# alshai/Big-BWT

Hardware: AMD Instinct MI355X
Metric: input MB/s to .bwt (bit-exact vs ref) (higher is better)
Workload: dtype u8; 1 GPU; BASELINE configs[2]: 64x mutated yeast-shaped FASTA (~0.79 GB), -w 10 -p 100, BWT + -s -e sampled SA; bytes_per_gpu=787308470, w=10, p=100, flags=6, phrases=16409159, words=921010, dict_bytes=79900101, parallelism=1 GPU

## Files before the change

big-bwt_amd/csrc/merge.hip:

```cpp
#include "kernels.hpp"
#include "prims.hpp"
#include "devutil.hpp"
#include <algorithm>
#include <cstdlib>

namespace pfp {

static constexpr int TB = 256;
constexpr int kOffTileLog = 11;


template <class I> struct alignas(16) Idx8 { I v[8]; };
__device__ __forceinline__ void tile_full_count(const uint32_t p8[8], int nk, uint64_t t0, uint32_t *__restrict__ tile_full,
                                                unsigned long long *__restrict__ first_full) {
  __shared__ uint32_t ws[4];
  uint32_t cfull = 0;
  int firstk = -1;
#pragma unroll
  for (int k = 7; k >= 0; k--) if (k < nk && p8[k] == kEndOfWord) { cfull++; firstk = k; }
  const unsigned long long anyf = __ballot(cfull != 0);
  for (int o = 32; o > 0; o >>= 1) cfull += __shfl_down(cfull, o, 64);
  if ((threadIdx.x & 63) == 0) ws[threadIdx.x >> 6] = cfull;
  if (anyf && (int)(threadIdx.x & 63) == __ffsll((long long)anyf) - 1) atomicMin(first_full, (unsigned long long)(t0 + firstk));
  __syncthreads();
// ... 169 lines not shown
__global__ void full_base0_kernel(const unsigned long long *__restrict__ first_full, const I *__restrict__ sa,
                                  WordView wv, const uint32_t *__restrict__ lexrank, uint32_t *__restrict__ out) {
  const unsigned long long f = *first_full;
  *out = f == ~0ull ? 0u : lexrank[word_of(wv, sa[f])];
}

template <class I>
__global__ void group_flags_kernel(uint64_t N, const I *__restrict__ grp, const uint8_t *__restrict__ pc,
                                   int any_multi_is_hard, uint8_t *__restrict__ hard) {
  uint64_t t = (uint64_t)BID * blockDim.x + threadIdx.x;
  if (t >= N || pc[t] == 0) return;
  I g = grp[t];
  if (g == t) return;
  if (any_multi_is_hard || pc[t] != pc[g]) hard[g] = 1;
}

enum : uint8_t { CLS_NONE = 0, CLS_FILL = 1, CLS_FULL = 2, CLS_HARD = 3, CLS_MULTI = 4 };
enum : int { SA_NONE = 0, SA_DENSE = 1, SA_SPARSE = 2 };

template <class I>
__global__ void gather_idx_kernel(uint64_t n, const I *__restrict__ idx, const I *__restrict__ src, I *__restrict__ dst) {
  uint64_t i = (uint64_t)BID * blockDim.x + threadIdx.x;
  if (i < n) dst[i] = src[idx[i]];
}
struct alignas(32) WordRec { uint32_t ist, occ, first, last; uint64_t wend, pad; };
__global__ void wistart_kernel(uint32_t d, const uint32_t *__restrict__ lexrank, const uint32_t *__restrict__ istart_lex,
                               const uint32_t *__restrict__ wocc, const uint32_t *__restrict__ ilist,
                               const uint64_t *__restrict__ wend, uint32_t *__restrict__ wistart, WordRec *__restrict__ wrec) {
  uint32_t j = BID * blockDim.x + threadIdx.x;
  if (j >= d) return;
  const uint32_t st = istart_lex[lexrank[j]] + 1;
  wistart[j] = st;
  if (wrec) { const uint32_t oc = wocc[j]; wrec[j] = WordRec{st, oc, ilist[st], ilist[st + oc - 1], wend[j], 0}; }
}

template <class I>
struct MergeArgsT {
  uint64_t N, n_out; uint32_t d; int w; int want_sa;
  uint64_t pos_base, n_out_global;
  uint64_t out_lo, out_hi;
  const I *sa, *grp;
  WordView wv;
  const uint32_t *ist, *wistart;
  const WordRec *wrec;
  const uint32_t *sfirst, *slast, *ssl;
  const uint8_t *pc, *hard, *gmaj;
  const uint64_t *tbase; const uint32_t *loc;
  const uint32_t *ilist; const uint8_t *bwlast; const uint64_t *bwsai;
  const uint32_t *istart_lex, *fullbase, *fullbase0;
  uint8_t *bwt; uint64_t *out_sa;
  int pass;
  const uint64_t *bmap, *bpre;
  uint64_t *sa_c;
};
enum : int { PASS_BWT = 1, PASS_SA = 2 };
template <class I>
__device__ __forceinline__ void sa_put(const MergeArgsT<I> &a, uint64_t x, uint64_t v) {
  if (x < a.out_lo || x >= a.out_hi) return;
  if (!a.bmap) { a.out_sa[x] = v; return; }
  const uint64_t r = x - a.out_lo, wv = a.bmap[r >> 6];
  if (!((wv >> (r & 63)) & 1ull)) return;
  if (a.sa_c) a.sa_c[a.bpre[r >> 6] + (uint64_t)__popcll(wv & ((1ull << (r & 63)) - 1ull))] = v;
  else a.out_sa[x] = v;
}
template <class I>
__device__ __forceinline__ bool sa_wanted(const MergeArgsT<I> &a, uint64_t x) {
  if (x < a.out_lo || x >= a.out_hi) return false;
  if (!a.bmap) return true;
  const uint64_t r = x - a.out_lo;
  return (a.bmap[r >> 6] >> (r & 63)) & 1ull;
}
template <class I>
__device__ __forceinline__ uint64_t slot_off(const MergeArgsT<I> &a, uint64_t t) { return a.tbase[t >> kOffTileLog] + a.loc[t]; }


__device__ __forceinline__ uint8_t fix_char(uint8_t ch) { return ch == kDollar ? 0 : ch; }
template <class I>
__device__ __forceinline__ uint32_t slot_ist(const MergeArgsT<I> &a, uint64_t t) {
  return a.ist ? a.ist[t] : a.wistart[word_of(a.wv, a.sa[t])];
}

template <class I>
__device__ __forceinline__ uint32_t slot_first(const MergeArgsT<I> &a, uint64_t t) { return a.sfirst ? a.sfirst[t] : a.wrec[word_of(a.wv, a.sa[t])].first; }
template <class I>
__device__ __forceinline__ uint32_t slot_last(const MergeArgsT<I> &a, uint64_t t) { return a.slast ? a.slast[t] : a.wrec[word_of(a.wv, a.sa[t])].last; }
template <class I>
__device__ __forceinline__ uint64_t slot_slen(const MergeArgsT<I> &a, uint64_t t) {
  if (a.ssl) { const uint32_t v = a.ssl[t]; if (v != kSlCap) return v; }
  return slen_of(a.wv, a.sa[t]);
}

constexpr int kHardLds = 1024;
constexpr int kHardRank = 512;
constexpr int kHardMem = 256;
constexpr int kHardSortMin = 512;
constexpr int kSlots = 2048;
constexpr uint64_t kExpandQuota = 1u << 16;

struct ExpandLds {
  uint32_t loff[kSlots + 1];
  uint32_t lfist[kSlots];
  uint8_t lpc[kSlots], lcls[kSlots];
  uint32_t ccnt[kSlots / 64 + 1];
};

template <class I>
// ... 383 lines not shown
          uint32_t lb, pv = 0, sv = 0;
          bool hp = false, hs = false;
          if (m == me) {
            lb = j;
            if (a.want_sa) {
              if (j > 0) { pv = a.ilist[my_ist + j - 1]; hp = true; }
              if (j + 1 < my_occ) { sv = a.ilist[my_ist + j + 1]; hs = true; }
            }
          } else {
            const uint32_t mfirst = slot_first(a, g + m), mlast = slot_last(a, g + m);
            if (pos < mfirst) { lb = 0; sv = mfirst; hs = true; }
            else if (pos > mlast) { lb = (uint32_t)(slot_off(a, g + m + 1) - slot_off(a, g + m)); pv = mlast; hp = true; }
            else {
              const WordRec wr = a.wrec[word_of(a.wv, a.sa[g + m])];
              const uint32_t *lst = a.ilist + wr.ist;
              uint32_t l2 = 1, h2 = wr.occ - 1;
              while (l2 < h2) { const uint32_t mid = (l2 + h2) >> 1; if (lst[mid] < pos) l2 = mid + 1; else h2 = mid; }
              lb = l2;
              if (a.want_sa) { pv = lst[lb - 1]; hp = true; sv = lst[lb]; hs = true; }
            }
          }
          r += lb;
          if (hp && (!has_pred || pv > pred)) { pred = pv; has_pred = 1; }
          if (hs && (!has_succ || sv < succ)) { succ = sv; has_succ = 1; }
        }
      }
#pragma unroll
      for (int o = 1; o < LPM; o <<= 1) {
        r += __shfl_xor(r, o, 64);
        const uint32_t op = __shfl_xor(pred, o, 64), ohp = __shfl_xor(has_pred, o, 64);
        const uint32_t os = __shfl_xor(succ, o, 64), ohs = __shfl_xor(has_succ, o, 64);
        if (ohp && (!has_pred || op > pred)) { pred = op; has_pred = 1; }
        if (ohs && (!has_succ || os < succ)) { succ = os; has_succ = 1; }
      }
      if (!act || ll != 0) continue;
      const uint64_t o = base + r;
      if (o >= a.out_lo && o < a.out_hi) a.bwt[o] = mych;
      if (a.want_sa)
        recs[mmv.roff + j] = MinorRec{o, pos, pred, succ, has_pred | (has_succ << 1), (uint32_t)sl, 0u};
    }
  }
}

template <class I>
__global__ void hard_minor_sa_kernel(MergeArgsT<I> a, const MinorRec *__restrict__ recs, uint64_t n) {
  const uint64_t q = (uint64_t)BID * blockDim.x + threadIdx.x;
  if (q >= n) return;
  const MinorRec r = recs[q];
  sa_put(a, r.o, a.bwsai[r.pos] - (uint64_t)r.sl);
  if ((r.flags & 1u) && r.o >= 1) sa_put(a, r.o - 1, a.bwsai[r.pred] - (uint64_t)r.sl);
  if (r.flags & 2u) sa_put(a, r.o + 1, a.bwsai[r.succ] - (uint64_t)r.sl);
}

struct BigGroup { uint64_t g; uint64_t E; uint32_t k; uint32_t pad; };
struct HardLds {
  uint32_t lpos[kHardRank];
  uint8_t lq[kHardRank];
  uint32_t lmoff[kHardMem + 1], lmist[kHardMem], lmsl[kHardMem];
  uint8_t lmch[kHardMem], lmg[kHardMem];
  uint64_t gbase[64], ghead[64];
  uint32_t geoff[65], gk0[65];
};
__device__ __forceinline__ void wave_lds_sync() {
  __builtin_amdgcn_wave_barrier();
  __threadfence_block();
}
__device__ __forceinline__ uint32_t wave_max_u32(uint32_t v) {
#pragma unroll
  for (int o = 32; o > 0; o >>= 1) { const uint32_t x = __shfl_xor(v, o, 64); v = x > v ? x : v; }
  return v;
}
template <class I>
__global__ __launch_bounds__(256) void hard_groups_kernel(MergeArgsT<I> a, const I *__restrict__ heads,
                                                          const uint64_t *__restrict__ nheads_p,
                                                          unsigned long long *__restrict__ stats,
                                                          BigGroup *__restrict__ big, uint32_t big_cap,
                                                          BigGroup *__restrict__ mid, uint32_t mid_cap, int gpb) {
  __shared__ HardLds S[4];
  const int wv = threadIdx.x >> 6, lane = threadIdx.x & 63;
  HardLds &L = S[wv];
  const uint64_t nH = *nheads_p;
  const uint64_t nbatch = (nH + gpb - 1) / gpb;
  unsigned long long my_chars = 0, my_groups = 0;
  for (uint64_t b = BID * 4 + wv; b < nbatch; b += GDIM * 4) {
    const uint64_t hidx = b * gpb + lane;
    uint64_t g = 0, base = 0;
    uint32_t k = 0, E = 0;
    bool live = false;
    if (lane < gpb && hidx < nH) {
      g = heads[hidx];
      uint32_t kk = 0;
      while (g + kk < a.N && a.grp[g + kk] == (I)g && a.pc[g + kk] != 0) kk++;
      base = slot_off(a, g);
      const uint64_t Eg = slot_off(a, g + kk) - base;
      if (kk && !(base + Eg <= a.out_lo || base >= a.out_hi)) {
        my_chars += Eg; my_groups += 1;
        const bool sorted_path = Eg > (uint64_t)kHardSortMin;
        if (Eg <= (uint64_t)kHardRank && kk <= (uint32_t)kHardMem && !sorted_path) { live = true; k = kk; E = (uint32_t)Eg; }
        else if (Eg <= (uint64_t)kHardLds && sorted_path) {
          const unsigned long long idx = atomicAdd(&stats[3], 1ull);
          if (idx < mid_cap) mid[idx] = BigGroup{g, Eg, kk, 0};
        } else {
          const unsigned long long idx = atomicAdd(&stats[2], 1ull);
          if (idx < big_cap) big[idx] = BigGroup{g, Eg, kk, 0};
        }
      }
    }
    unsigned long long todo = __ballot(live);
    while (todo) {
      const bool mine = (todo >> lane) & 1ull;
      uint32_t pk = mine ? k : 0u, pE = mine ? E : 0u;
#pragma unroll
      for (int o = 1; o < 64; o <<= 1) {
        const uint32_t vk = __shfl_up(pk, o, 64), vE = __shfl_up(pE, o, 64);
        if (lane >= o) { pk += vk; pE += vE; }
      }
      const bool fit = mine && pk <= (uint32_t)kHardMem && pE <= (uint32_t)kHardRank;
      const unsigned long long take = __ballot(fit);
      todo &= ~take;
      const int nG = __popcll(take);
      const int lastl = 63 - __clzll((long long)take);
      const uint32_t M = __shfl(pk, lastl, 64), Eb = __shfl(pE, lastl, 64);
      if (fit) {
        const int gi = __popcll(take & ((1ull << lane) - 1ull));
        L.ghead[gi] = g; L.gbase[gi] = base; L.geoff[gi] = pE - E; L.gk0[gi] = pk - k;
      }
      if (lane == 0) { L.geoff[nG] = Eb; L.gk0[nG] = M; }
      wave_lds_sync();
      for (uint32_t q = lane; q < M; q += 64) {
        int lo = 0, hi = nG;
        while (hi - lo > 1) { const int mid = (lo + hi) >> 1; if (L.gk0[mid] <= q) lo = mid; else hi = mid; }
        const uint64_t t = L.ghead[lo] + (q - L.gk0[lo]);
        L.lmoff[q] = L.geoff[lo] + (uint32_t)(slot_off(a, t) - L.gbase[lo]);
        L.lmist[q] = slot_ist(a, t);
        uint32_t sl = 0;
        if (a.want_sa) sl = (uint32_t)slot_slen(a, t);
        L.lmsl[q] = sl;
        L.lmch[q] = fix_char(a.pc[t]);
        L.lmg[q] = (uint8_t)lo;
      }
      if (lane == 0) L.lmoff[M] = Eb;
      wave_lds_sync();
      for (uint32_t e = lane; e < Eb; e += 64) {
        uint32_t lo = 0, hi = M;
        while (hi - lo > 1) { const uint32_t mid = (lo + hi) >> 1; if (L.lmoff[mid] <= e) lo = mid; else hi = mid; }
        L.lpos[e] = a.ilist[L.lmist[lo] + (e - L.lmoff[lo])];
        L.lq[e] = (uint8_t)lo;
      }
      wave_lds_sync();
      for (uint32_t e = lane; e < Eb; e += 64) {
        const uint32_t q = L.lq[e], gi = L.lmg[q];
        const uint32_t s0 = L.geoff[gi], s1 = L.geoff[gi + 1], k0 = L.gk0[gi], k1 = L.gk0[gi + 1];
        const uint32_t Eg = s1 - s0, kg = k1 - k0;
        const uint32_t pos = L.lpos[e];
        uint32_t lg = 1;
        while ((kg << lg) < Eg) lg++;
        const bool by_search = (uint64_t)kg * (lg + 1) * 3 < Eg;
        uint32_t r = 0;
        if (!by_search) {
          for (uint32_t x = s0; x < s1; x++) r += L.lpos[x] < pos;
        } else {
          for (uint32_t m2 = k0; m2 < k1; m2++) {
            uint32_t l2 = L.lmoff[m2], h2 = L.lmoff[m2 + 1];
            const uint32_t b2 = l2;
            while (l2 < h2) { const uint32_t mid = (l2 + h2) >> 1; if (L.lpos[mid] < pos) l2 = mid + 1; else h2 = mid; }
            r += l2 - b2;
          }
        }
        const uint64_t o = L.gbase[gi] + r;
        if (o >= a.out_lo && o < a.out_hi) {
          if (a.pass & PASS_BWT) a.bwt[o] = L.lmch[q];
          if (a.want_sa && (a.pass & PASS_SA)) sa_put(a, o, a.bwsai[pos] - (uint64_t)L.lmsl[q]);
        }
      }
      wave_lds_sync();
    }
  }
#pragma unroll
  for (int o = 32; o > 0; o >>= 1) { my_chars += __shfl_down(my_chars, o, 64); my_groups += __shfl_down(my_groups, o, 64); }
  if (lane == 0 && (my_chars | my_groups)) { atomicAdd(&stats[0], my_chars); atomicAdd(&stats[1], my_groups); }
}

template <class I>
__global__ __launch_bounds__(256) void hard_sort_kernel(MergeArgsT<I> a, const BigGroup *__restrict__ mid, uint32_t nmid) {
  __shared__ uint64_t skey[4][kHardLds];
  const int wv = threadIdx.x >> 6, lane = threadIdx.x & 63;
  uint64_t *K = skey[wv];
  for (uint32_t qi = BID * 4 + wv; qi < nmid; qi += GDIM * 4) {
    const uint64_t g = mid[qi].g;
    const uint32_t E = (uint32_t)mid[qi].E, k = mid[qi].k;
    const uint64_t base = slot_off(a, g);
    uint32_t n = 64;
    while (n < E) n <<= 1;
    for (uint32_t e = lane; e < n; e += 64) {
      uint64_t key = ~0ull;
      if (e < E) {
        uint32_t lo = 0, hi = k;
        while (hi - lo > 1) { const uint32_t mdl = (lo + hi) >> 1; if (slot_off(a, g + mdl) - base <= e) lo = mdl; else hi = mdl; }
        const uint32_t pos = a.ilist[slot_ist(a, g + lo) + (e - (uint32_t)(slot_off(a, g + lo) - base))];
        key = ((uint64_t)pos << 16) | e;
      }
      K[e] = key;
    }
    wave_lds_sync();
    for (uint32_t k2 = 2; k2 <= n; k2 <<= 1)
      for (uint32_t j = k2 >> 1; j > 0; j >>= 1) {
        for (uint32_t i = lane; i < (n >> 1); i += 64) {
          const uint32_t x = ((i & ~(j - 1)) << 1) | (i & (j - 1)), y = x | j;
          const uint64_t kx = K[x], ky = K[y];
          if ((kx > ky) == ((x & k2) == 0)) { K[x] = ky; K[y] = kx; }
        }
        wave_lds_sync();
      }
    for (uint32_t r = lane; r < E; r += 64) {
      const uint64_t key = K[r];
      const uint32_t pos = (uint32_t)(key >> 16), e = (uint32_t)(key & 0xffffu);
      const uint64_t o = base + r;
      if (o < a.out_lo || o >= a.out_hi) continue;
      uint32_t lo = 0, hi = k;
      while (hi - lo > 1) { const uint32_t mdl = (lo + hi) >> 1; if (slot_off(a, g + mdl) - base <= e) lo = mdl; else hi = mdl; }
      const uint64_t t = g + lo;
      if (a.pass & PASS_BWT) a.bwt[o] = fix_char(a.pc[t]);
      if (a.want_sa && (a.pass & PASS_SA)) sa_put(a, o, a.bwsai[pos] - slot_slen(a, t));
    }
    wave_lds_sync();
  }
}

template <class I>
__global__ __launch_bounds__(256) void hard_big_kernel(MergeArgsT<I> a, const BigGroup *__restrict__ big, uint32_t nbig,
                                                       const uint64_t *__restrict__ estart, uint64_t total) {
  const uint64_t e0 = estart[0];
  for (uint64_t gi = (uint64_t)BID * 256 + threadIdx.x; gi < total; gi += (uint64_t)GDIM * 256) {
    const uint64_t ge = e0 + gi;
    uint32_t lo = 0, hi = nbig;
    while (hi - lo > 1) { uint32_t mid = (lo + hi) >> 1; if (estart[mid] <= ge) lo = mid; else hi = mid; }
    const uint64_t g = big[lo].g, e = ge - estart[lo];
    const uint32_t k = big[lo].k;
    const uint64_t base = slot_off(a, g);
    uint32_t ml = 0, mh = k;
    while (mh - ml > 1) { uint32_t mid = (ml + mh) >> 1; if (slot_off(a, g + mid) - base <= e) ml = mid; else mh = mid; }
    const uint64_t t = g + ml;
    const uint32_t j = (uint32_t)(e - (slot_off(a, t) - base));
    const uint32_t pos = a.ilist[slot_ist(a, t) + j];
    uint64_t r = j;
    for (uint64_t t2 = g; t2 < g + k; t2++) {
      if (t2 == t) continue;
      const uint32_t *lst = a.ilist + slot_ist(a, t2);
      uint32_t l2 = 0, h2 = (uint32_t)(slot_off(a, t2 + 1) - slot_off(a, t2));
      while (l2 < h2) { uint32_t mid = (l2 + h2) >> 1; if (lst[mid] < pos) l2 = mid + 1; else h2 = mid; }
      r += l2;
    }
    if (base + r >= a.out_lo && base + r < a.out_hi) {
      if (a.pass & PASS_BWT) a.bwt[base + r] = fix_char(a.pc[t]);
      if (a.want_sa && (a.pass & PASS_SA)) sa_put(a, base + r, a.bwsai[pos] - slot_slen(a, t));
    }
  }
}

template <class I>
__global__ __launch_bounds__(256) void big_keys_kernel(MergeArgsT<I> a, const BigGroup *__restrict__ big, uint32_t q0, uint32_t q1,
                                                       const uint64_t *__restrict__ estart, uint64_t cnt,
                                                       uint64_t *__restrict__ keys, uint64_t *__restrict__ vals) {
  const uint64_t i = (uint64_t)BID * 256 + threadIdx.x;
  if (i >= cnt) return;
  const uint64_t ge = estart[q0] + i;
  uint32_t lo = q0, hi = q1;
  while (hi - lo > 1) { const uint32_t mid = (lo + hi) >> 1; if (estart[mid] <= ge) lo = mid; else hi = mid; }
  const uint64_t g = big[lo].g, e = ge - estart[lo];
  const uint32_t k = big[lo].k;
  const uint64_t base = slot_off(a, g);
  uint32_t ml = 0, mh = k;
  while (mh - ml > 1) { const uint32_t mid = (ml + mh) >> 1; if (slot_off(a, g + mid) - base <= e) ml = mid; else mh = mid; }
  const uint64_t t = g + ml;
  const uint32_t j = (uint32_t)(e - (slot_off(a, t) - base));
  keys[i] = ((uint64_t)(lo - q0) << 32) | a.ilist[slot_ist(a, t) + j];
  vals[i] = t;
}
template <class I>
__global__ __launch_bounds__(256) void big_place_kernel(MergeArgsT<I> a, const BigGroup *__restrict__ big, uint32_t q0,
                                                        const uint64_t *__restrict__ estart, uint64_t cnt,
                                                        const uint64_t *__restrict__ keys, const uint64_t *__restrict__ vals) {
  const uint64_t i = (uint64_t)BID * 256 + threadIdx.x;
  if (i >= cnt) return;
  const uint64_t key = keys[i], t = vals[i];
  const uint32_t lo = q0 + (uint32_t)(key >> 32), pos = (uint32_t)key;
  const uint64_t o = slot_off(a, big[lo].g) + (estart[q0] + i - estart[lo]);
  if (o < a.out_lo || o >= a.out_hi) return;
  if (a.pass & PASS_BWT) a.bwt[o] = fix_char(a.pc[t]);
  if (a.want_sa && (a.pass & PASS_SA) && sa_wanted(a, o)) sa_put(a, o, a.bwsai[pos] - slot_slen(a, t));
}

__global__ __launch_bounds__(256) void slot_loc_kernel(const uint32_t *__restrict__ cnt, uint64_t N, uint32_t *__restrict__ loc,
                                                       uint64_t *__restrict__ tsum, uint32_t *__restrict__ overflow) {
  __shared__ uint64_t ws[4];
  if (((uint64_t)BID << kOffTileLog) > N) return;
  const uint64_t t0 = ((uint64_t)BID << kOffTileLog) + (uint64_t)threadIdx.x * 8;
  uint32_t v[8];
  if (t0 + 8 <= N) {
    const uint4 x = *reinterpret_cast<const uint4 *>(cnt + t0), y = *reinterpret_cast<const uint4 *>(cnt + t0 + 4);
    v[0] = x.x; v[1] = x.y; v[2] = x.z; v[3] = x.w; v[4] = y.x; v[5] = y.y; v[6] = y.z; v[7] = y.w;
  } else {
    for (int k = 0; k < 8; k++) v[k] = t0 + k < N ? cnt[t0 + k] : 0u;
  }
  uint64_t own = 0;
  for (int k = 0; k < 8; k++) own += v[k];
  uint64_t inc = own;
  const int lane = threadIdx.x & 63, wv = threadIdx.x >> 6;
  for (int o = 1; o < 64; o <<= 1) { const uint64_t u = __shfl_up(inc, o, 64); if (lane >= o) inc += u; }
  if (lane == 63) ws[wv] = inc;
  __syncthreads();
  uint64_t run = inc - own;
  for (int q = 0; q < wv; q++) run += ws[q];
  uint32_t o8[8];
  for (int k = 0; k < 8; k++) { o8[k] = (uint32_t)run; run += v[k]; }
  *reinterpret_cast<uint4 *>(loc + t0) = make_uint4(o8[0], o8[1], o8[2], o8[3]);
  *reinterpret_cast<uint4 *>(loc + t0 + 4) = make_uint4(o8[4], o8[5], o8[6], o8[7]);
  if (threadIdx.x == 255) {
    tsum[BID] = run;
    if (run >> 32) atomicOr(overflow, 1u);
  }
}


enum class RecordSource {
  SortKeys,
  Gathered,
  PerSlot,
};

struct MergeSwitches {
  int prec_direct = -1;
  uint32_t big_cap = 0;
  uint64_t big_budget = 1ull << 27;
  static MergeSwitches read() {
    MergeSwitches s;
    if (const char *e = getenv("PFP_PREC_DIRECT")) s.prec_direct = atoi(e) != 0;
    if (const char *e = getenv("PFP_BIG_CAP")) { if (atoll(e) > 0) s.big_cap = (uint32_t)atoll(e); }
    if (const char *e = getenv("PFP_BIG_BUDGET")) s.big_budget = strtoull(e, nullptr, 10);
    return s;
  }
};

// ... 20 lines not shown
  const Dictionary &D;
  const DictIndex &ix;
  const SuffixOrderT<I> &so;
  const ParseBWT &pb;
  const uint32_t *const occ_lex;
  const MergeOpts o;
  BwtOutputs &out;
  const uint64_t NP, N;
  const uint32_t d;
  const int sa_mode;
  const MergeSwitches sw;
  const RecordSource src;
  const WordView wv;
  const uint64_t ntile;
  const uint32_t nblk;
  const int first_pass;

  MergeArgsT<I> a{};
  uint64_t n_out = 0;

  struct {
    DBuf<uint32_t> istart_lex, wistart;
    DBuf<WordRec> wrec;
  } word;
  struct {
    DBuf<uint8_t> pc, hard;
    DBuf<uint32_t> loc, ovf;
    DBuf<uint64_t> tsum, tbase;
    DBuf<uint32_t> tile_full, fullbase, fullbase0;
    DBuf<unsigned long long> first_full;
    DBuf<uint32_t> sfirst, slast, ssl;
  } slot;
  enum { kAllHeads = 0, kFallbackHeads = 1 };
  struct {
    DBuf<unsigned long long> hstats;
    uint64_t n_heads = 0;
    uint32_t big_cap = 0, mid_cap = 0;
    DBuf<BigGroup> big, mid;
    DBuf<I> heads;
    DBuf<uint64_t> list_len;
    DBuf<unsigned long long> mstat;
    DBuf<uint8_t> gmaj, fallback;
    DBuf<HardGroupInfo> ginfo;
    DBuf<uint32_t> minor_cnt, mm_cnt;
    DBuf<uint64_t> minor_off, mm_off;
    DBuf<MinorMember> mm_list;
    uint64_t n_mm = 0, sum_k = 0, n_minor = 0;
    DBuf<I> fb_heads;
    DBuf<MinorRec> recs;
    int gpb = 64;
    uint32_t nmid = 0, nbig = 0;
    DBuf<uint64_t> estart;
    std::vector<uint64_t> es;
  } hg;
  DBuf<uint32_t> heavy, nheavy;

  Merge(pfp_ctx *c_, const Dictionary &D_, const DictIndex &ix_, const SuffixOrderT<I> &so_, const ParseBWT &pb_, const uint32_t *occ_lex_,
        const MergeOpts &o_, BwtOutputs &out_)
      : c(c_), D(D_), ix(ix_), so(so_), pb(pb_), occ_lex(occ_lex_), o(o_), out(out_), NP(D_.dsize), N(so_.N), d((uint32_t)D_.d),
        sa_mode(!o_.flags ? SA_NONE : ((o_.flags & PFP_FLAG_SA) ? SA_DENSE : SA_SPARSE)), sw(MergeSwitches::read()),
        src(choose_record_source<I>(c_, N, NP, sa_mode, so_, sw)), wv(word_view(D_, ix_)), ntile((N >> kOffTileLog) + 1),
        nblk((uint32_t)cdiv64(N, kSlots)), first_pass(sa_mode == SA_SPARSE ? PASS_BWT : (PASS_BWT | PASS_SA)) {}

  MergeArgsT<I> with_pass(int pass) const { MergeArgsT<I> x = a; x.pass = pass; return x; }

  void word_records() {
    word.istart_lex.alloc(c, d); word.wistart.alloc(c, d);
    exclusive_sum_u32(c, occ_lex, word.istart_lex.p, d);
    word.wrec.alloc(c, d);
    hipLaunchKernelGGL(wistart_kernel, gdim(cdiv(d, TB)), gdim(TB), 0, c->stream, d, ix.lexrank.p, word.istart_lex.p, D.wocc.p, pb.ilist.p,
                       ix.wend.p, word.wistart.p, word.wrec.p);
  }

  void alloc_slot_tables() {
    slot.pc.alloc(c, N + 8); slot.hard.alloc(c, N);
    slot.loc.alloc(c, ntile << kOffTileLog); slot.ovf.alloc(c, 1);
    alloc_counts(c, slot.tsum, ntile); slot.tbase.alloc(c, ntile + 1);
    slot.hard.zero();
    slot.tile_full.alloc(c, ntile + 1); slot.fullbase.alloc(c, ntile + 1); slot.fullbase0.alloc(c, 1);
    slot.first_full.alloc(c, 1);
    slot.tile_full.zero();
    PFP_HIP(hipMemsetAsync(slot.first_full.p, 0xFF, 8, c->stream));
    slot.ovf.zero();
  }
  void slot_tables_from_keys(DBuf<uint32_t> &cnt) {
    { KScope ks(c, "pfp::slot_payload_kernel", N * (8 + 1 + 5));
      hipLaunchKernelGGL(slot_payload_kernel<I>, gdim(cdiv(cdiv64(N, 8), 256)), gdim(256), 0, c->stream, N, so.sa.p, so.skeys.p,
                         so.refined.p, D.bytes.p, wv, D.wocc.p, d, o.w, cnt.p, slot.pc.p, slot.tile_full.p, slot.first_full.p); }
    { KScope ks(c, "pfp::slot_loc_kernel", N * 8);
      hipLaunchKernelGGL(slot_loc_kernel, gdim((unsigned)ntile), gdim(256), 0, c->stream, cnt.p, N, slot.loc.p, slot.tsum.p, slot.ovf.p); }
    { KScope ks(c, "pfp::group_flags_kernel", N * 5);
      hipLaunchKernelGGL(group_flags_kernel<I>, gdim(cdiv(N, TB)), gdim(TB), 0, c->stream, N, so.grp.p, slot.pc.p, 0, slot.hard.p); }
  }
  void slot_tables_gathered() {
    const int dense = sa_mode == SA_DENSE ? 1 : 0;
    const uint64_t np256 = cdiv64(NP, 256) * 256;
    DBuf<PosRec> prec(c, np256);
    { KScope ks(c, "pfp::pprec16_kernel", NP * (1 + 16) + (uint64_t)d * 40);
      hipLaunchKernelGGL(pprec16_kernel, gdim(cdiv(np256, TB)), gdim(TB), 0, c->stream, wv, o.w, reinterpret_cast<const uint4 *>(word.wrec.p),
                         dense, (uint64_t)0, NP, prec.p); }
    slot_records(prec.p);
  }
  void slot_tables_per_slot() { slot_records(nullptr); }
  void slot_records(const PosRec *prec) {
    const int dense = sa_mode == SA_DENSE ? 1 : 0;
    slot.sfirst.alloc(c, ntile << kOffTileLog);
// ... 25 lines not shown
    a.ist = dense ? slot.sfirst.p : nullptr;
    a.wistart = word.wistart.p; a.wrec = word.wrec.p;
    a.sfirst = dense ? nullptr : slot.sfirst.p; a.slast = slot.slast.p; a.ssl = slot.ssl.p;
    a.pc = slot.pc.p; a.hard = slot.hard.p; a.tbase = slot.tbase.p; a.loc = slot.loc.p;
    a.ilist = pb.ilist.p; a.bwlast = pb.bwlast.p; a.bwsai = pb.bwsai.p;
    a.istart_lex = word.istart_lex.p; a.fullbase = slot.fullbase.p; a.fullbase0 = slot.fullbase0.p;
    a.out_lo = o.out_lo; a.out_hi = o.out_hi < n_out ? o.out_hi : n_out;
    a.bwt = out.d_bwt - o.out_lo; a.out_sa = out.d_sa ? out.d_sa - o.out_lo : nullptr;
  }

  void find_hard_groups() {
    hg.hstats.alloc(c, 5);
    hg.hstats.zero();
    hg.n_heads = count_flags(c, slot.hard.p, N);
    hg.big_cap = sw.big_cap ? sw.big_cap : (uint32_t)std::min<uint64_t>({(uint64_t)1u << 20, hg.n_heads + 1, n_out / 1024 + 1});
    hg.big.alloc(c, hg.big_cap);
    hg.mid_cap = (uint32_t)std::min<uint64_t>(n_out / (kHardSortMin + 1) + 64, 0x7FFFFFFFull);
    hg.mid.alloc(c, hg.mid_cap);
    hg.heads.alloc(c, hg.n_heads + 1);
    hg.list_len.alloc(c, 2);
    select_index<I>(c, slot.hard.p, hg.heads.p, hg.list_len.p + kAllHeads, N);
    hg.mstat.alloc(c, 2);
    hg.mstat.zero();
  }

  HeadList<I> classify() {
    const uint64_t n_heads = hg.n_heads;
    hg.gmaj.alloc(c, N); hg.fallback.alloc(c, n_heads); hg.ginfo.alloc(c, n_heads);
    alloc_counts(c, hg.minor_cnt, n_heads); hg.minor_off.alloc(c, n_heads + 1);
    alloc_counts(c, hg.mm_cnt, n_heads); hg.mm_off.alloc(c, n_heads + 1);
    a.gmaj = hg.gmaj.p;
    { KScope ks(c, "pfp::hard_classify_kernel", n_heads * 40);
      hipLaunchKernelGGL(hard_classify_kernel<I>, gdim(cdiv(n_heads, 256)), gdim(256), 0, c->stream, a, hg.heads.p, n_heads, hg.gmaj.p,
                         hg.ginfo.p, hg.minor_cnt.p, hg.fallback.p, hg.mstat.p, hg.mm_cnt.p); }
    exclusive_sum_u32_u64(c, hg.minor_cnt.p, hg.minor_off.p, n_heads + 1);
    exclusive_sum_u32_u64(c, hg.mm_cnt.p, hg.mm_off.p, n_heads + 1);
    hg.n_mm = read_scalar(c, hg.mm_off.p + n_heads);
    hg.sum_k = read_scalar(c, (const uint64_t *)hg.mstat.p + 1);
    if (hg.n_mm) {
      hg.mm_list.alloc(c, hg.n_mm);
      KScope ks(c, "pfp::hard_minor_fill_kernel", n_heads * 40 + hg.n_mm * 16);
      hipLaunchKernelGGL(hard_minor_fill_kernel<I>, gdim(cdiv(n_heads * 8, 256)), gdim(256), 0, c->stream, a, hg.ginfo.p, n_heads, hg.mm_off.p,
                         hg.minor_off.p, hg.gmaj.p, hg.mm_list.p);
    }
    const uint64_t n_fallback = count_flags(c, hg.fallback.p, n_heads);
    hg.n_minor = read_scalar(c, hg.minor_off.p + n_heads);
    hg.fb_heads.alloc(c, n_fallback + 1);
    {
      DBuf<I> fidx(c, n_fallback + 1);
      select_index<I>(c, hg.fallback.p, fidx.p, hg.list_len.p + kFallbackHeads, n_heads);
      if (n_fallback) hipLaunchKernelGGL(gather_idx_kernel<I>, gdim(cdiv(n_fallback, 256)), gdim(256), 0, c->stream, n_fallback, fidx.p,
                                         hg.heads.p, hg.fb_heads.p);
      PFP_HIP(hipGetLastError());
      sync(c);
    }
    return HeadList<I>{hg.fb_heads.p, hg.list_len.p + kFallbackHeads, n_fallback};
  }

  void expand() {
    const MergeArgsT<I> ap = with_pass(first_pass);
    heavy.alloc(c, nblk); nheavy.alloc(c, 1);
    nheavy.zero();
    { KScope ks(c, "pfp::expand_kernel", N * 14 + n_out * (sa_mode == SA_DENSE ? 17 : 1));
      hipLaunchKernelGGL(expand_kernel<I>, gdim(nblk), gdim(256), 0, c->stream, ap, heavy.p, nheavy.p, nblk); }
    const uint32_t nh = read_scalar(c, nheavy.p);
    KScope ks2(c, "pfp::expand_heavy_kernel", 0);
    if (nh) hipLaunchKernelGGL(expand_heavy_kernel<I>, gdim(c->n_cu * 4), gdim(256), 0, c->stream, ap, heavy.p, nh);
    PFP_HIP(hipGetLastError());
  }

  void place_minority(const HeadList<I> &lds) {
    if (hg.n_mm) {
      const MergeArgsT<I> ap = with_pass(first_pass);
      if (sa_mode == SA_SPARSE) hg.recs.alloc(c, hg.n_minor + 1);
      KScope ks(c, "pfp::hard_minor_kernel", hg.n_minor * 64);
      const uint64_t avg_k = hg.sum_k / std::max<uint64_t>(hg.n_heads - lds.n, 1);
      if (avg_k > 32)
        hipLaunchKernelGGL((hard_minor_kernel<I, 64>), gdim((unsigned)std::min<uint64_t>(cdiv64(hg.n_mm, 4), (uint64_t)c->n_cu * 64)), gdim(256), 0,
                           c->stream, ap, hg.mm_list.p, hg.n_mm, hg.recs.p);
      else
        hipLaunchKernelGGL((hard_minor_kernel<I, 8>), gdim((unsigned)std::min<uint64_t>(cdiv64(hg.n_mm, 32), (uint64_t)c->n_cu * 64)), gdim(256), 0,
                           c->stream, ap, hg.mm_list.p, hg.n_mm, hg.recs.p);
    }
    PFP_HIP(hipGetLastError());
  }

  void rank_in_lds(const HeadList<I> &lds) {
    const MergeArgsT<I> ap = with_pass(first_pass);
    while (hg.gpb > 8 && lds.n / hg.gpb < (uint64_t)c->n_cu * 32) hg.gpb >>= 1;
    for (;;) {
      if (!lds.n) { PFP_HIP(hipMemsetAsync(hg.hstats.p, 0, 40, c->stream)); }
      else { KScope ks(c, "pfp::hard_groups_kernel", N * 5);
        hipLaunchKernelGGL(hard_groups_kernel<I>, gdim(c->n_cu * 8), gdim(256), 0, c->stream, ap, lds.heads, lds.n_dev, hg.hstats.p, hg.big.p,
                           hg.big_cap, hg.mid.p, hg.mid_cap, hg.gpb); }
      PFP_HIP(hipGetLastError());
      PFP_HIP(hipMemcpyAsync(c->h_scalars, hg.hstats.p, 40, hipMemcpyDeviceToHost, c->stream));
      sync(c);
      if (c->h_scalars[2] <= hg.big_cap) break;
      hg.big_cap = (uint32_t)std::min<uint64_t>(c->h_scalars[2], 0xFFFFFFFFull);
      hg.big.alloc(c, hg.big_cap);
      hg.hstats.zero();
    }
    out.hard_chars = c->h_scalars[0];
    out.hard_groups = c->h_scalars[1];
    out.hard_minor_groups = hg.n_heads - lds.n; out.hard_minor_chars = hg.n_minor;
    out.hard_big_groups = c->h_scalars[2]; out.hard_max_members = c->h_scalars[4];
    hg.nmid = (uint32_t)std::min<uint64_t>(c->h_scalars[3], hg.mid_cap);
    PFP_REQUIRE(c->h_scalars[3] <= hg.mid_cap, PFP_EHIP, "more sorted-path hard groups than the output can hold");
    hg.nbig = (uint32_t)c->h_scalars[2];
    out.hard_chars += read_scalar(c, (const uint64_t *)hg.mstat.p);
    out.hard_groups += hg.n_heads - lds.n;
  }

  void lay_out_queued() {
    const uint32_t nbig = hg.nbig;
    hg.es.assign(nbig + 1, 0);
    if (!nbig) return;
    std::vector<BigGroup> hb(nbig);
    PFP_HIP(hipMemcpyAsync(hb.data(), hg.big.p, nbig * sizeof(BigGroup), hipMemcpyDeviceToHost, c->stream));
    sync(c);
    for (uint32_t q = 0; q < nbig; q++) hg.es[q + 1] = hg.es[q] + hb[q].E;
    hg.estart.alloc(c, nbig + 1);
    PFP_HIP(hipMemcpyAsync(hg.estart.p, hg.es.data(), (nbig + 1) * 8, hipMemcpyHostToDevice, c->stream));
    sync(c);
  }

  void queued_groups(int pass) {
    const MergeArgsT<I> ap = with_pass(pass);
    const std::vector<uint64_t> &es = hg.es;
    if (hg.nmid) {
      KScope ks(c, "pfp::hard_sort_kernel", (uint64_t)hg.nmid * (kHardSortMin + 1) * (sa_mode ? 21 : 5));
      hipLaunchKernelGGL(hard_sort_kernel<I>, gdim(c->n_cu * 4), gdim(256), 0, c->stream, ap, hg.mid.p, hg.nmid);
      PFP_HIP(hipGetLastError());
    }
    for (uint32_t q0 = 0; q0 < hg.nbig;) {
      uint32_t q1 = q0 + 1;
      while (q1 < hg.nbig && es[q1 + 1] - es[q0] <= sw.big_budget) q1++;
      const uint64_t cnt = es[q1] - es[q0];
      if (cnt > sw.big_budget) {
        const int nb = (int)std::min<uint64_t>(cdiv64(cnt, 256), (uint64_t)c->n_cu * 32);
        KScope ks(c, "pfp::hard_big_kernel", cnt * (sa_mode ? 21 : 5));
        hipLaunchKernelGGL(hard_big_kernel<I>, gdim(nb), gdim(256), 0, c->stream, ap, hg.big.p + q0, q1 - q0, hg.estart.p + q0, cnt);
      } else {
        DBuf<uint64_t> bk(c, cnt), bka(c, cnt), bv(c, cnt), bva(c, cnt);
        { KScope ks(c, "pfp::big_keys_kernel", cnt * 28);
          hipLaunchKernelGGL(big_keys_kernel<I>, gdim(cdiv(cnt, 256)), gdim(256), 0, c->stream, ap, hg.big.p, q0, q1, hg.estart.p, cnt, bk.p, bv.p); }
        { SortTag tag("large hard groups"); sort_pairs_db<uint64_t, uint64_t>(c, bk, bka, bv, bva, cnt, 0, 32 + bits_for(q1 - q0)); }
        { KScope ks(c, "pfp::big_place_kernel", cnt * (sa_mode ? 34 : 18));
          hipLaunchKernelGGL(big_place_kernel<I>, gdim(cdiv(cnt, 256)), gdim(256), 0, c->stream, ap, hg.big.p, q0, hg.estart.p, cnt, bk.p, bv.p); }
      }
      PFP_HIP(hipGetLastError());
      q0 = q1;
    }
  }

  void mark_run_boundaries() {
    const uint64_t cnt_slice = a.out_hi > a.out_lo ? a.out_hi - a.out_lo : 0;
    const uint64_t nw = cdiv64(cnt_slice, 64);
    out.bmap.alloc(c, nw + 1); out.bpre.alloc(c, nw + 1);
    const bool want_s = !out.d_sa && (o.flags & PFP_FLAG_SSA), want_e = !out.d_sa && (o.flags & PFP_FLAG_ESA);
    out.slice_n = cnt_slice;
    {
      DBuf<uint32_t> wcnt, scnt, ecnt;
      alloc_counts(c, wcnt, nw);
      PFP_HIP(hipMemsetAsync(out.bmap.p + nw, 0, 8, c->stream));
      if (want_s) { out.smap.alloc(c, nw + 1); out.spre.alloc(c, nw + 1); alloc_counts(c, scnt, nw); }
      if (want_e) { out.emap.alloc(c, nw + 1); out.epre.alloc(c, nw + 1); alloc_counts(c, ecnt, nw); }
      if (nw) {
        KScope ks(c, "pfp::run_bitmap_kernel", cnt_slice + nw * (12 + (want_s ? 12 : 0) + (want_e ? 12 : 0)));
        hipLaunchKernelGGL(run_bitmap_kernel, gdim(cdiv(cdiv64(cnt_slice, 16), 256)), gdim(256), 0, c->stream, out.d_bwt, cnt_slice,
                           out.bmap.p, wcnt.p, out.smap.p, scnt.p, out.emap.p, ecnt.p);
      }
      exclusive_sum_u32_u64(c, wcnt.p, out.bpre.p, nw + 1);
      if (want_s) exclusive_sum_u32_u64(c, scnt.p, out.spre.p, nw + 1);
      if (want_e) exclusive_sum_u32_u64(c, ecnt.p, out.epre.p, nw + 1);
      out.n_bound = read_scalar(c, out.bpre.p + nw);
      if (want_s) out.n_starts = read_scalar(c, out.spre.p + nw);
      if (want_e) out.n_ends = read_scalar(c, out.epre.p + nw);
    }
    a.bmap = out.bmap.p; a.bpre = out.bpre.p;
    if (!out.d_sa) {
      out.sa_c.alloc(c, out.n_bound + 1);
      if (c->debug) PFP_HIP(hipMemsetAsync(out.sa_c.p, 0xFF, (out.n_bound + 1) * 8, c->stream));
      a.sa_c = out.sa_c.p;
    }
  }

  void sa_round(const HeadList<I> &lds) {
    const MergeArgsT<I> ap = with_pass(PASS_SA);
    PFP_REQUIRE(ix.wslot_lex.p, PFP_EINVAL, "merge: the dictionary index has no whole-word slots (compute_lexrank has not run)");
    if (pb.P) {
      KScope ks(c, "pfp::word_sa_kernel", pb.P * (4 + 8 + 8 + 8));
      hipLaunchKernelGGL(word_sa_kernel<I>, gdim(cdiv(pb.P, 256)), gdim(256), 0, c->stream, ap, pb.P, ix.wslot_lex.p, so.slot_base);
    }
    { KScope ks(c, "pfp::unit_edges_kernel", N * (1 + sizeof(I) * 2 + 4));
      hipLaunchKernelGGL(unit_edges_kernel<I>, gdim(cdiv(N, 256)), gdim(256), 0, c->stream, ap); }
    if (hg.n_mm) {
      const uint64_t nr = hg.n_minor;
      if (nr) hipLaunchKernelGGL(hard_minor_sa_kernel<I>, gdim(cdiv(nr, 256)), gdim(256), 0, c->stream, ap, hg.recs.p, nr);
    }
    if (lds.n) {
      DBuf<unsigned long long> scratch(c, 5);
      scratch.zero();
      KScope ks(c, "pfp::hard_groups_kernel", N * 5);
      hipLaunchKernelGGL(hard_groups_kernel<I>, gdim(c->n_cu * 8), gdim(256), 0, c->stream, ap, lds.heads, lds.n_dev, scratch.p, hg.big.p,
                         0u, hg.mid.p, 0u, hg.gpb);
      PFP_HIP(hipGetLastError());
      queued_groups(PASS_SA);
      sync(c);
    }
    PFP_HIP(hipGetLastError());
  }

  void check_boundaries_set() {
    if (!c->debug || !a.sa_c) return;
    DBuf<unsigned long long> unset(c, 1);
    unset.zero();
    const uint64_t skip_lo = (a.pos_base + a.out_lo > 0) ? 1 : 0, skip_hi = (a.pos_base + a.out_hi < a.n_out_global) ? 1 : 0;
    if (out.n_bound > skip_lo + skip_hi)
      hipLaunchKernelGGL(count_unset_kernel, gdim(cdiv(out.n_bound, 256)), gdim(256), 0, c->stream, out.sa_c.p + skip_lo,
                         out.n_bound - skip_lo - skip_hi, unset.p);
    const uint64_t u = read_scalar(c, (const uint64_t *)unset.p);
    PFP_REQUIRE(u == 0, PFP_EHIP, "sparse SA: " + std::to_string(u) + " run boundaries of the BWT received no SA value");
  }

  void run() {
    PFP_REQUIRE(!o.flags || pb.bwsai.p, PFP_EINVAL, "SA output requested without sa info");
    word_records();
    {
      DBuf<uint32_t> cnt;
      if (src == RecordSource::SortKeys) alloc_counts(c, cnt, N, 8);
      alloc_slot_tables();
      switch (src) {
        case RecordSource::SortKeys: slot_tables_from_keys(cnt); break;
        case RecordSource::Gathered: slot_tables_gathered(); break;
        case RecordSource::PerSlot: slot_tables_per_slot(); break;
      }
      offsets_and_totals();
    }
    fill_args();
    find_hard_groups();
    const HeadList<I> lds = sa_mode != SA_DENSE && hg.n_heads ? classify() : HeadList<I>{hg.heads.p, hg.list_len.p + kAllHeads, hg.n_heads};
    expand();
    place_minority(lds);
    rank_in_lds(lds);
    lay_out_queued();
    queued_groups(first_pass);
    if (sa_mode == SA_SPARSE) {
      mark_run_boundaries();
      sa_round(lds);
      check_boundaries_set();
    }
    sync(c);
  }
};

template <class I>
void merge_bwt(pfp_ctx *c, const Dictionary &D, const DictIndex &ix, const SuffixOrderT<I> &so, const ParseBWT &pb,
               const uint32_t *occ_lex, const MergeOpts &o, BwtOutputs &out) {
  Merge<I>(c, D, ix, so, pb, occ_lex, o, out).run();
}
template void merge_bwt<uint32_t>(pfp_ctx *, const Dictionary &, const DictIndex &, const SuffixOrderT<uint32_t> &, const ParseBWT &,
                                  const uint32_t *, const MergeOpts &, BwtOutputs &);
template void merge_bwt<uint64_t>(pfp_ctx *, const Dictionary &, const DictIndex &, const SuffixOrderT<uint64_t> &, const ParseBWT &,
                                  const uint32_t *, const MergeOpts &, BwtOutputs &);

}
```

Before: 26010 MB/s.

## Record hard-group ranked positions in first pass and reuse them for sparse SA

The first pass over hard groups now records each group's ranked text position into a compact buffer (hpos, indexed by a prefix sum hoff over the listed groups). The sparse-SA round then reads those stored positions through a new chunked hard_sa_kernel instead of rerunning hard_groups_kernel and the queued sort/big kernels. This removes a second full ranking pass, which repeats searches, sorts and LDS work. In exchange it adds an index build with a scalar readback, extra global writes of positions during the first pass, and temporary memory of four bytes per hard character.

```diff
diff --git a/big-bwt_amd/csrc/merge.hip b/big-bwt_amd/csrc/merge.hip
--- a/big-bwt_amd/csrc/merge.hip
+++ b/big-bwt_amd/csrc/merge.hip
@@ -245,6 +245,8 @@
   int pass;
   const uint64_t *bmap, *bpre;
   uint64_t *sa_c;
+  const uint64_t *hoff;
+  uint32_t *hpos;
 };
 enum : int { PASS_BWT = 1, PASS_SA = 2 };
 template <class I>
@@ -734,7 +736,7 @@
   if (r.flags & 2u) sa_put(a, r.o + 1, a.bwsai[r.succ] - (uint64_t)r.sl);
 }
 
-struct BigGroup { uint64_t g; uint64_t E; uint32_t k; uint32_t pad; };
+struct BigGroup { uint64_t g; uint64_t E; uint32_t k; uint32_t pad; uint64_t hoff; };
 struct HardLds {
   uint32_t lpos[kHardRank];
   uint8_t lq[kHardRank];
@@ -742,6 +744,7 @@
   uint8_t lmch[kHardMem], lmg[kHardMem];
   uint64_t gbase[64], ghead[64];
   uint32_t geoff[65], gk0[65];
+  uint8_t glane[64];
 };
 __device__ __forceinline__ void wave_lds_sync() {
   __builtin_amdgcn_wave_barrier();
@@ -781,10 +784,10 @@
         if (Eg <= (uint64_t)kHardRank && kk <= (uint32_t)kHardMem && !sorted_path) { live = true; k = kk; E = (uint32_t)Eg; }
         else if (Eg <= (uint64_t)kHardLds && sorted_path) {
           const unsigned long long idx = atomicAdd(&stats[3], 1ull);
-          if (idx < mid_cap) mid[idx] = BigGroup{g, Eg, kk, 0};
+          if (idx < mid_cap) mid[idx] = BigGroup{g, Eg, kk, 0, a.hoff ? a.hoff[hidx] : 0ull};
         } else {
           const unsigned long long idx = atomicAdd(&stats[2], 1ull);
-          if (idx < big_cap) big[idx] = BigGroup{g, Eg, kk, 0};
+          if (idx < big_cap) big[idx] = BigGroup{g, Eg, kk, 0, a.hoff ? a.hoff[hidx] : 0ull};
         }
       }
     }
@@ -806,6 +809,7 @@
       if (fit) {
         const int gi = __popcll(take & ((1ull << lane) - 1ull));
         L.ghead[gi] = g; L.gbase[gi] = base; L.geoff[gi] = pE - E; L.gk0[gi] = pk - k;
+        L.glane[gi] = (uint8_t)lane;
       }
       if (lane == 0) { L.geoff[nG] = Eb; L.gk0[nG] = M; }
       wave_lds_sync();
@@ -815,9 +819,7 @@
         const uint64_t t = L.ghead[lo] + (q - L.gk0[lo]);
         L.lmoff[q] = L.geoff[lo] + (uint32_t)(slot_off(a, t) - L.gbase[lo]);
         L.lmist[q] = slot_ist(a, t);
-        uint32_t sl = 0;
-        if (a.want_sa) sl = (uint32_t)slot_slen(a, t);
-        L.lmsl[q] = sl;
+        if (a.want_sa == SA_DENSE) L.lmsl[q] = (uint32_t)slot_slen(a, t);
         L.lmch[q] = fix_char(a.pc[t]);
         L.lmg[q] = (uint8_t)lo;
       }
@@ -850,9 +852,10 @@
           }
         }
         const uint64_t o = L.gbase[gi] + r;
+        if (a.hpos) a.hpos[a.hoff[b * gpb + L.glane[gi]] + r] = pos;
         if (o >= a.out_lo && o < a.out_hi) {
-          if (a.pass & PASS_BWT) a.bwt[o] = L.lmch[q];
-          if (a.want_sa && (a.pass & PASS_SA)) sa_put(a, o, a.bwsai[pos] - (uint64_t)L.lmsl[q]);
+          a.bwt[o] = L.lmch[q];
+          if (a.want_sa == SA_DENSE) sa_put(a, o, a.bwsai[pos] - (uint64_t)L.lmsl[q]);
         }
       }
       wave_lds_sync();
@@ -871,7 +874,7 @@
   for (uint32_t qi = BID * 4 + wv; qi < nmid; qi += GDIM * 4) {
     const uint64_t g = mid[qi].g;
     const uint32_t E = (uint32_t)mid[qi].E, k = mid[qi].k;
-    const uint64_t base = slot_off(a, g);
+    const uint64_t base = slot_off(a, g), ho = mid[qi].hoff;
     uint32_t n = 64;
     while (n < E) n <<= 1;
     for (uint32_t e = lane; e < n; e += 64) {
@@ -898,12 +901,13 @@
       const uint64_t key = K[r];
       const uint32_t pos = (uint32_t)(key >> 16), e = (uint32_t)(key & 0xffffu);
       const uint64_t o = base + r;
+      if (a.hpos) a.hpos[ho + r] = pos;
       if (o < a.out_lo || o >= a.out_hi) continue;
       uint32_t lo = 0, hi = k;
       while (hi - lo > 1) { const uint32_t mdl = (lo + hi) >> 1; if (slot_off(a, g + mdl) - base <= e) lo = mdl; else hi = mdl; }
       const uint64_t t = g + lo;
-      if (a.pass & PASS_BWT) a.bwt[o] = fix_char(a.pc[t]);
-      if (a.want_sa && (a.pass & PASS_SA)) sa_put(a, o, a.bwsai[pos] - slot_slen(a, t));
+      a.bwt[o] = fix_char(a.pc[t]);
+      if (a.want_sa == SA_DENSE) sa_put(a, o, a.bwsai[pos] - slot_slen(a, t));
     }
     wave_lds_sync();
   }
@@ -933,9 +937,10 @@
       while (l2 < h2) { uint32_t mid = (l2 + h2) >> 1; if (lst[mid] < pos) l2 = mid + 1; else h2 = mid; }
       r += l2;
     }
+    if (a.hpos) a.hpos[big[lo].hoff + r] = pos;
     if (base + r >= a.out_lo && base + r < a.out_hi) {
-      if (a.pass & PASS_BWT) a.bwt[base + r] = fix_char(a.pc[t]);
-      if (a.want_sa && (a.pass & PASS_SA)) sa_put(a, base + r, a.bwsai[pos] - slot_slen(a, t));
+      a.bwt[base + r] = fix_char(a.pc[t]);
+      if (a.want_sa == SA_DENSE) sa_put(a, base + r, a.bwsai[pos] - slot_slen(a, t));
     }
   }
 }
@@ -967,10 +972,58 @@
   if (i >= cnt) return;
   const uint64_t key = keys[i], t = vals[i];
   const uint32_t lo = q0 + (uint32_t)(key >> 32), pos = (uint32_t)key;
-  const uint64_t o = slot_off(a, big[lo].g) + (estart[q0] + i - estart[lo]);
+  const uint64_t r = estart[q0] + i - estart[lo];
+  const uint64_t o = slot_off(a, big[lo].g) + r;
+  if (a.hpos) a.hpos[big[lo].hoff + r] = pos;
   if (o < a.out_lo || o >= a.out_hi) return;
-  if (a.pass & PASS_BWT) a.bwt[o] = fix_char(a.pc[t]);
-  if (a.want_sa && (a.pass & PASS_SA) && sa_wanted(a, o)) sa_put(a, o, a.bwsai[pos] - slot_slen(a, t));
+  a.bwt[o] = fix_char(a.pc[t]);
+  if (a.want_sa == SA_DENSE) sa_put(a, o, a.bwsai[pos] - slot_slen(a, t));
+}
+
+template <class I>
+__global__ void hard_index_kernel(uint64_t nq, const I *__restrict__ fidx, const HardGroupInfo *__restrict__ info,
+                                  uint64_t *__restrict__ E) {
+  const uint64_t q = (uint64_t)BID * blockDim.x + threadIdx.x;
+  if (q < nq) E[q] = info[fidx[q]].E;
+}
+constexpr int kSaChunk = 2048;
+__global__ void hard_sa_starts_kernel(const uint64_t *__restrict__ hoff, uint64_t nq, uint64_t H, uint64_t nchunk,
+                                      uint64_t *__restrict__ bstart) {
+  const uint64_t b = (uint64_t)BID * blockDim.x + threadIdx.x;
+  if (b > nchunk) return;
+  const uint64_t x = b * kSaChunk < H ? b * kSaChunk : H - 1;
+  uint64_t lo = 0, hi = nq;
+  while (hi - lo > 1) { const uint64_t mid = (lo + hi) >> 1; if (hoff[mid] <= x) lo = mid; else hi = mid; }
+  bstart[b] = lo;
+}
+template <class I>
+__global__ __launch_bounds__(256) void hard_sa_kernel(MergeArgsT<I> a, const I *__restrict__ heads, uint64_t H,
+                                                      const uint64_t *__restrict__ bstart) {
+  __shared__ uint64_t lh[257], lbase[256], lsl[256];
+  const uint64_t x0 = (uint64_t)BID * kSaChunk;
+  if (x0 >= H) return;
+  const uint64_t x1 = x0 + kSaChunk < H ? x0 + kSaChunk : H;
+  const uint64_t q0 = bstart[BID], q1 = bstart[BID + 1];
+  for (uint64_t qb = q0; qb <= q1; qb += 256) {
+    const int nw = q1 - qb + 1 >= 256 ? 256 : (int)(q1 - qb + 1);
+    __syncthreads();
+    if ((int)threadIdx.x < nw) {
+      const uint64_t g = heads[qb + threadIdx.x];
+      lh[threadIdx.x] = a.hoff[qb + threadIdx.x];
+      lbase[threadIdx.x] = slot_off(a, g);
+      lsl[threadIdx.x] = slot_slen(a, g);
+    }
+    if (threadIdx.x == 0) lh[nw] = a.hoff[qb + nw];
+    __syncthreads();
+    const uint64_t wlo = lh[0], whi = lh[nw];
+    for (uint64_t x = x0 + threadIdx.x; x < x1; x += 256) {
+      if (x < wlo || x >= whi) continue;
+      int lo = 0, hi = nw;
+      while (hi - lo > 1) { const int mid = (lo + hi) >> 1; if (lh[mid] <= x) lo = mid; else hi = mid; }
+      const uint64_t o = lbase[lo] + (x - lh[lo]);
+      if (sa_wanted(a, o)) sa_put(a, o, a.bwsai[a.hpos[x]] - lsl[lo]);
+    }
+  }
 }
 
 __global__ __launch_bounds__(256) void slot_loc_kernel(const uint32_t *__restrict__ cnt, uint64_t N, uint32_t *__restrict__ loc,
@@ -1097,6 +1150,9 @@
     uint32_t nmid = 0, nbig = 0;
     DBuf<uint64_t> estart;
     std::vector<uint64_t> es;
+    DBuf<uint64_t> hoff;
+    DBuf<uint32_t> hpos;
+    uint64_t H = 0;
   } hg;
   DBuf<uint32_t> heavy, nheavy;
 
@@ -1228,9 +1284,22 @@
       if (n_fallback) hipLaunchKernelGGL(gather_idx_kernel<I>, gdim(cdiv(n_fallback, 256)), gdim(256), 0, c->stream, n_fallback, fidx.p,
                                          hg.heads.p, hg.fb_heads.p);
       PFP_HIP(hipGetLastError());
-      sync(c);
+      if (sa_mode == SA_SPARSE && n_fallback) index_listed_groups(fidx.p, n_fallback);
+      else sync(c);
     }
     return HeadList<I>{hg.fb_heads.p, hg.list_len.p + kFallbackHeads, n_fallback};
+  }
+
+  void index_listed_groups(const I *fidx, uint64_t nq) {
+    DBuf<uint64_t> E;
+    alloc_counts(c, E, nq);
+    hg.hoff.alloc(c, nq + 1);
+    hipLaunchKernelGGL(hard_index_kernel<I>, gdim(cdiv(nq, 256)), gdim(256), 0, c->stream, nq, fidx, hg.ginfo.p, E.p);
+    PFP_HIP(hipGetLastError());
+    exclusive_sum_u64(c, E.p, hg.hoff.p, nq + 1);
+    hg.H = read_scalar(c, hg.hoff.p + nq);
+    hg.hpos.alloc(c, hg.H);
+    a.hoff = hg.hoff.p; a.hpos = hg.hpos.p;
   }
 
   void expand() {
@@ -1301,11 +1370,12 @@
     sync(c);
   }
 
-  void queued_groups(int pass) {
-    const MergeArgsT<I> ap = with_pass(pass);
+  void queued_groups() {
+    const MergeArgsT<I> ap = with_pass(first_pass);
     const std::vector<uint64_t> &es = hg.es;
+    const uint64_t sa_bytes = sa_mode == SA_DENSE ? 16 : (sa_mode == SA_SPARSE ? 4 : 0);
     if (hg.nmid) {
-      KScope ks(c, "pfp::hard_sort_kernel", (uint64_t)hg.nmid * (kHardSortMin + 1) * (sa_mode ? 21 : 5));
+      KScope ks(c, "pfp::hard_sort_kernel", (uint64_t)hg.nmid * (kHardSortMin + 1) * (5 + sa_bytes));
       hipLaunchKernelGGL(hard_sort_kernel<I>, gdim(c->n_cu * 4), gdim(256), 0, c->stream, ap, hg.mid.p, hg.nmid);
       PFP_HIP(hipGetLastError());
     }
@@ -1315,14 +1385,14 @@
       const uint64_t cnt = es[q1] - es[q0];
       if (cnt > sw.big_budget) {
         const int nb = (int)std::min<uint64_t>(cdiv64(cnt, 256), (uint64_t)c->n_cu * 32);
-        KScope ks(c, "pfp::hard_big_kernel", cnt * (sa_mode ? 21 : 5));
+        KScope ks(c, "pfp::hard_big_kernel", cnt * (5 + sa_bytes));
         hipLaunchKernelGGL(hard_big_kernel<I>, gdim(nb), gdim(256), 0, c->stream, ap, hg.big.p + q0, q1 - q0, hg.estart.p + q0, cnt);
       } else {
         DBuf<uint64_t> bk(c, cnt), bka(c, cnt), bv(c, cnt), bva(c, cnt);
         { KScope ks(c, "pfp::big_keys_kernel", cnt * 28);
           hipLaunchKernelGGL(big_keys_kernel<I>, gdim(cdiv(cnt, 256)), gdim(256), 0, c->stream, ap, hg.big.p, q0, q1, hg.estart.p, cnt, bk.p, bv.p); }
         { SortTag tag("large hard groups"); sort_pairs_db<uint64_t, uint64_t>(c, bk, bka, bv, bva, cnt, 0, 32 + bits_for(q1 - q0)); }
-        { KScope ks(c, "pfp::big_place_kernel", cnt * (sa_mode ? 34 : 18));
+        { KScope ks(c, "pfp::big_place_kernel", cnt * (18 + sa_bytes));
           hipLaunchKernelGGL(big_place_kernel<I>, gdim(cdiv(cnt, 256)), gdim(256), 0, c->stream, ap, hg.big.p, q0, hg.estart.p, cnt, bk.p, bv.p); }
       }
       PFP_HIP(hipGetLastError());
@@ -1375,17 +1445,18 @@
       const uint64_t nr = hg.n_minor;
       if (nr) hipLaunchKernelGGL(hard_minor_sa_kernel<I>, gdim(cdiv(nr, 256)), gdim(256), 0, c->stream, ap, hg.recs.p, nr);
     }
-    if (lds.n) {
-      DBuf<unsigned long long> scratch(c, 5);
-      scratch.zero();
-      KScope ks(c, "pfp::hard_groups_kernel", N * 5);
-      hipLaunchKernelGGL(hard_groups_kernel<I>, gdim(c->n_cu * 8), gdim(256), 0, c->stream, ap, lds.heads, lds.n_dev, scratch.p, hg.big.p,
-                         0u, hg.mid.p, 0u, hg.gpb);
+    if (hg.H) {
+      const uint64_t nchunk = cdiv64(hg.H, kSaChunk);
+      DBuf<uint64_t> bstart(c, nchunk + 1);
+      KScope ks(c, "pfp::hard_sa_kernel", hg.H * 4 + cdiv64(hg.H, 64) * 8 + lds.n * (sizeof(I) + 8 + 12) + (nchunk + 1) * 8);
+      hipLaunchKernelGGL(hard_sa_starts_kernel, gdim(cdiv(nchunk + 1, 256)), gdim(256), 0, c->stream, hg.hoff.p, lds.n, hg.H, nchunk, bstart.p);
+      hipLaunchKernelGGL(hard_sa_kernel<I>, gdim(nchunk), gdim(256), 0, c->stream, ap, lds.heads, hg.H, bstart.p);
       PFP_HIP(hipGetLastError());
-      queued_groups(PASS_SA);
       sync(c);
     }
     PFP_HIP(hipGetLastError());
+    a.hoff = nullptr; a.hpos = nullptr;
+    hg.hpos.release(); hg.hoff.release();
   }
 
   void check_boundaries_set() {
@@ -1421,7 +1492,7 @@
     place_minority(lds);
     rank_in_lds(lds);
     lay_out_queued();
-    queued_groups(first_pass);
+    queued_groups();
     if (sa_mode == SA_SPARSE) {
       mark_run_boundaries();
       sa_round(lds);
```

Result: faster. 26670 MB/s (median of 6 runs) (+2.5%).
